# OpenVVC/OpenVVC

Hardware: AMD Instinct MI355X
Metric: decoded frames/sec, full rcn back-end decode step (H2D of the recorded picture + MC incl. BDOF/DMVR/affine-PROF/GPM/CIIP + LMCS + inverse transform + ordered intra pass + deblocking + SAO + ALF/CC-ALF + D2H of refined MVs + wait + per-picture digest + publication to the device DPB), 4K 10-bit RA rec (higher is better)
Workload: dtype u16 samples / int16 coefficients / int32 accumulate

## Files before the change

include/ovvc_hip.h:

```cpp
#ifndef OVVC_HIP_H
#define OVVC_HIP_H

#include <stddef.h>
#include <stdint.h>

#ifdef __cplusplus
extern "C" {
#endif

#define OVHIP_ABI_VERSION 9

#define OVHIP_OK        0
#define OVHIP_ENODEV   (-1)
#define OVHIP_ENOMEM   (-2)
#define OVHIP_EINVAL   (-3)
#define OVHIP_ELAUNCH  (-4)
#define OVHIP_EUNSUP   (-5)
#define OVHIP_EREF     (-6)

enum { OVHIP_DST_VII = 0, OVHIP_DCT_VIII = 1, OVHIP_DCT_II = 2 };

typedef struct ovhip_pic {
    uint16_t *y, *cb, *cr;
    int32_t   w, h;
// ... 557 lines not shown
                       const ovhip_aff_unit *d_aunits, uint32_t n_aunits, const int32_t *d_side,
                       const uint16_t *d_lmcs_fwd_lut);
#define OVHIP_INTRA_GEOM_ANY 0x12u
#define OVHIP_INTRA_GEOM_IBC 0x20u
uint32_t ovhip_intra_level_geom(const ovhip_itask *tasks, size_t n);
int  ovhip_intra_level_launch(ovhip_ctx *ctx, const ovhip_pic *pic, const ovhip_pic *res, const ovhip_itask *d_tasks, uint32_t n,
                              const ovhip_lmcs_region *d_regions, const ovhip_lmcs_luts *luts, int16_t *d_scales, int32_t log2_ctu_s,
                              uint32_t geom);
size_t ovhip_intra_sync_words(int32_t width, int32_t height, int32_t log2_ctu_s);
int  ovhip_intra_ctu_launch(ovhip_ctx *ctx, const ovhip_pic *pic, const ovhip_pic *res, const ovhip_itask *d_tasks, const ovhip_ictu *d_ctus,
                            uint32_t n_ctus, const ovhip_lmcs_region *d_regions, const ovhip_lmcs_luts *luts, int16_t *d_scales,
                            int32_t log2_ctu_s, uint32_t *d_sync, uint32_t epoch, uint32_t *abort_mirror);
#define OVHIP_FLOW_IBC 2
size_t ovhip_intra_flow_words(int32_t width, int32_t height);
size_t ovhip_intra_flow_items(const ovhip_itask *sorted, size_t n, uint32_t *items, size_t cap);
int  ovhip_intra_flow_launch(ovhip_ctx *ctx, const ovhip_pic *pic, const ovhip_pic *res, const ovhip_itask *d_tasks, uint32_t n_tasks,
                             const uint32_t *d_items, uint32_t n_items, const ovhip_lmcs_region *d_regions, const ovhip_lmcs_luts *luts,
                             int16_t *d_scales, int32_t log2_ctu_s, uint32_t *d_state, uint32_t epoch, uint32_t *abort_mirror, int32_t prepare,
                             int32_t n_workers);
int  ovhip_intra_flow_untag_launch(ovhip_ctx *ctx, const ovhip_pic *pic, const ovhip_itask *d_tasks, uint32_t n_tasks, int32_t with_luma);
int  ovhip_lmcs_scale_prepare_launch(ovhip_ctx *ctx, const ovhip_pic *pic, const ovhip_lmcs_region *d_regions, uint32_t n_regions,
                                     const ovhip_lmcs_luts *luts, int16_t *d_scales, const ovhip_itask *d_tasks, uint32_t n_tasks,
                                     uint32_t *d_state, uint32_t epoch);
int  ovhip_lmcs_inverse_untag_launch(ovhip_ctx *ctx, const ovhip_pic *pic, const uint16_t *d_bwd_lut, const ovhip_itask *d_tasks, uint32_t n_tasks);
int  ovhip_dbf_launch(ovhip_ctx *ctx, const ovhip_pic *pic, const ovhip_dbf_planes *planes);
int  ovhip_dbf_launch_edges(ovhip_ctx *ctx, const ovhip_pic *pic, const ovhip_dbf_edge *d_edges_v, uint32_t n_v,
                            const ovhip_dbf_edge *d_edges_h, uint32_t n_h, int32_t beta_offset, int32_t tc_offset);
int  ovhip_dbf_launch_edges_ex(ovhip_ctx *ctx, const ovhip_pic *pic, const ovhip_dbf_edge *d_edges_v, uint32_t n_v,
                               const ovhip_dbf_edge *d_edges_h, uint32_t n_h, const ovhip_dbf_offsets *offsets);
int  ovhip_sao_launch(ovhip_ctx *ctx, const ovhip_pic *dst, const ovhip_pic *src,
// ... 452 lines not shown
```

openvvc_amd/capi.py:

```python
from __future__ import annotations

import ctypes as C
import os
from pathlib import Path

import numpy as np

_PKG = Path(__file__).resolve().parent
LIB_PATH = _PKG / os.environ.get("OVVC_HIP_LIB_NAME", "libovvc_hip.so")

OVHIP_ABI_VERSION = 9
OVHIP_OK, OVHIP_ENODEV, OVHIP_ENOMEM, OVHIP_EINVAL, OVHIP_ELAUNCH, OVHIP_EUNSUP, OVHIP_EREF = 0, -1, -2, -3, -4, -5, -6
DST_VII, DCT_VIII, DCT_II = 0, 1, 2
TB_TR, TB_DC, TB_TS, TB_TS_RAW = 0, 1, 2, 3
TB_FLAG_RASTER = 0x80
RES_ADD, RES_SUB, RES_ADD_HALF, RES_SUB_HALF, RES_SCALE = 0, 1, 2, 3, 4
MC_HPEL_FILT, MC_FILT_4x4, MC_NO_LUMA, MC_NO_CHROMA, MC_LMCS, MC_BDOF, MC_DMVR = 1, 2, 4, 8, 16, 32, 64
PU_BDOF, PU_DMVR, PU_GPM = 1, 2, 4
MC_GPM = 128


class Pic(C.Structure):
    _fields_ = [("y", C.c_void_p), ("cb", C.c_void_p), ("cr", C.c_void_p),
                ("w", C.c_int32), ("h", C.c_int32), ("stride_y", C.c_int32), ("stride_c", C.c_int32)]
# ... 580 lines not shown
        "ovhip_mcx_launch": (C.c_int, [vp, P(Pic), P(Pic), u32, vp, u32, vp, vp]),
        "ovhip_mca_launch": (C.c_int, [vp, P(Pic), P(Pic), u32, vp, u32, vp, vp]),
        "ovhip_mcxa_launch": (C.c_int, [vp, P(Pic), P(Pic), u32, vp, u32, vp, vp, u32, vp, vp]),
        "ovhip_rec_create_ex": (vp, [i32, i32, vp]),
        "ovhip_rec_set_dense_dbf_planes": (None, [vp, C.c_int]),
        "ovhip_rec_dbf_edges": (vp, [vp, C.c_int, P(C.c_size_t), P(DbfOffsets)]),
        "ovhip_dbf_launch_edges_ex": (C.c_int, [vp, P(Pic), vp, u32, vp, u32, P(DbfOffsets)]),
        "ovhip_dmvr_search_launch": (C.c_int, [vp, P(Pic), P(Pic), u32, vp, u32, vp]),
        "ovhip_rec_append_raw": (C.c_int, [vp, C.c_int, vp, C.c_size_t]),
        "ovhip_itx_launch_classes_res": (C.c_int, [vp, P(Pic), P(Pic), vp, u32, u32, vp, vp]),
        "ovhip_intra_level_launch": (C.c_int, [vp, P(Pic), P(Pic), vp, u32, vp, vp, vp, i32, u32]),
        "ovhip_intra_level_geom": (u32, [vp, C.c_size_t]),
        "ovhip_intra_sync_words": (C.c_size_t, [i32, i32, i32]),
        "ovhip_intra_flow_words": (C.c_size_t, [i32, i32]),
        "ovhip_intra_flow_items": (C.c_size_t, [vp, C.c_size_t, vp, C.c_size_t]),
        "ovhip_intra_flow_launch": (C.c_int, [vp, P(Pic), P(Pic), vp, u32, vp, u32, vp, vp, vp, i32, vp, u32, vp, i32, i32]),
        "ovhip_intra_ctu_launch": (C.c_int, [vp, P(Pic), P(Pic), vp, vp, u32, vp, vp, vp, i32, vp, u32, vp]),
        "ovhip_rec_itask_levels": (u32, [vp]),
        "ovhip_rec_isp_cu": (C.c_int, [vp, vp, vp]),
        "ovhip_isp_geometry": (None, [i32, i32, i32, P(i32), P(i32), P(i32), P(i32)]),
        "ovhip_job_bind": (C.c_int, [vp, vp]),
        "ovhip_rec_set_ctu_size": (C.c_int, [vp, i32]),
        "ovhip_rec_itasks_by_ctu": (vp, [vp, i32, P(C.c_size_t), P(vp), P(C.c_size_t)]),
        "ovhip_rec_tu_intra": (C.c_int, [vp, P(TuState), P(TuDesc), P(ITask), P(ITask)]),
        "ovhip_rec_itasks": (vp, [vp, P(C.c_size_t)]),
        "ovhip_rec_ibc_check": (C.c_int, [vp, P(IbcDesc)]),
        "ovhip_rec_tu_ibc": (C.c_int, [vp, P(TuState), P(TuDesc), P(IbcDesc)]),
        "ovhip_rec_ibc_tasks": (C.c_size_t, [vp]),
        "ovhip_rec_itasks_sorted": (vp, [vp, P(C.c_size_t), P(P(C.c_uint32)), P(C.c_uint32)]),
        "ovhip_rec_set_dbf_offsets": (C.c_int, [vp, P(DbfOffsets), C.c_int]),
# ... 193 lines not shown
        raise RuntimeError("libovvc_hip.so ABI version mismatch")
    if path is None:
        _lib = lib
    return lib


EXPORTED_SYMBOLS = [
    "ovhip_abi_version", "ovhip_rec_create", "ovhip_rec_destroy", "ovhip_rec_reset", "ovhip_rec_tu",
    "ovhip_rec_pu", "ovhip_rec_cu_inter", "ovhip_rec_dbf_row", "ovhip_rec_dbf_mv_prepass_view", "ovhip_rec_dbf_ctu", "ovhip_rec_dbf_planes", "ovhip_dbf_launch", "ovhip_sao_launch", "ovhip_alf_launch", "ovhip_rec_tb_cmds", "ovhip_rec_coefs", "ovhip_rec_mc_units", "ovhip_rec_mcx_units", "ovhip_mcx_launch", "ovhip_rec_affine_cu", "ovhip_rec_transform_tree", "ovhip_rec_lmcs_region", "ovhip_dbf_compact", "ovhip_rec_dbf_mv_prepass", "ovhip_dbf_launch_edges", "ovhip_rec_ciip", "ovhip_ciip_weight", "ovhip_rec_ciip_units", "ovhip_ciip_launch", "ovhip_rec_lmcs_regions", "ovhip_rec_tb_cmds_split", "ovhip_itx_launch_classes", "ovhip_itx_launch_chroma_lmcs", "ovhip_lmcs_build", "ovhip_lmcs_scale_launch", "ovhip_lmcs_inverse_launch", "ovhip_rec_aff_units", "ovhip_rec_aff_side", "ovhip_mca_launch", "ovhip_mcxa_launch", "ovhip_ctx_create",
    "ovhip_ctx_destroy", "ovhip_ctx_sync", "ovhip_ctx_shares_queue", "ovhip_ctx_new_stream", "ovhip_ctx_fork", "ovhip_ctx_join", "ovhip_last_error", "ovhip_ctx_stream", "ovhip_malloc",
    "ovhip_free", "ovhip_h2d", "ovhip_d2h", "ovhip_pic_alloc", "ovhip_pic_free", "ovhip_pic_upload",
    "ovhip_pic_download", "ovhip_itx_launch", "ovhip_mc_launch",
    "ovhip_rec_set_ref_scale", "ovhip_rec_refusal", "ovhip_rec_rpr_units", "ovhip_mc_rpr_launch",
    "ovhip_rec_set_rpr_tools", "ovhip_rec_aff_rpr_units", "ovhip_mca_rpr_launch",
    "ovhip_rec_create_ex", "ovhip_rec_set_dense_dbf_planes", "ovhip_rec_dbf_edges", "ovhip_dbf_launch_edges_ex",
    "ovhip_dmvr_search_launch", "ovhip_rec_append_raw", "ovhip_rec_set_dbf_offsets", "ovhip_rec_tu_intra", "ovhip_rec_itasks", "ovhip_rec_itasks_sorted", "ovhip_itx_launch_classes_res", "ovhip_intra_level_launch", "ovhip_intra_level_geom", "ovhip_intra_sync_words", "ovhip_intra_ctu_launch", "ovhip_intra_flow_words", "ovhip_intra_flow_items", "ovhip_intra_flow_launch",
    "ovhip_rec_itask_levels", "ovhip_rec_isp_cu", "ovhip_isp_geometry", "ovhip_rec_itasks_by_ctu", "ovhip_rec_set_ctu_size", "ovhip_job_bind", "ovhip_job_create", "ovhip_job_destroy", "ovhip_job_recorder", "ovhip_job_begin",
    "ovhip_frame_band", "ovhip_frame_band_upto", "ovhip_frame_dmvr_rows_begin_upto", "ovhip_job_dmvr_rows_begin_upto", "ovhip_frame_set_band_mode", "ovhip_frame_band_stats", "ovhip_dpb_post_rows", "ovhip_dpb_rows_tag",
    "ovhip_job_band", "ovhip_job_band_active", "ovhip_job_band_busy", "ovhip_job_band_reserve", "ovhip_job_reserve_for_picture", "ovhip_rec_reserve_for_picture", "ovhip_job_band_progress", "ovhip_rec_counts", "ovhip_sao_launch_rows", "ovhip_alf_launch_rows",
    "ovhip_job_flush", "ovhip_job_wait", "ovhip_job_refined_mvs", "ovhip_job_dmvr_rows", "ovhip_job_dmvr_rows_begin", "ovhip_job_dmvr_rows_collect", "ovhip_job_last_stats", "ovhip_job_time_stage", "ovhip_job_stage_time",
    "ovhip_output_bytes", "ovhip_output_rows", "ovhip_output_pack_launch", "ovhip_output_row_md5_launch", "ovhip_output_bands", "ovhip_output_tree_md5_launch", "ovhip_pic_output", "ovhip_pic_digest",
    "ovhip_md5_init", "ovhip_md5_update", "ovhip_md5_final", "ovhip_tmvp_cells_launch", "ovhip_job_tmvp_cells", "ovhip_intra_flow_untag_launch", "ovhip_lmcs_inverse_untag_launch", "ovhip_lmcs_scale_prepare_launch",
    "ovhip_host_alloc", "ovhip_host_free", "ovhip_d2d", "ovhip_job_test_abort_next_flow",
    "ovhip_dpb_create", "ovhip_dpb_create_ex", "ovhip_dpb_destroy", "ovhip_dpb_n_devices", "ovhip_dpb_device", "ovhip_dpb_begin", "ovhip_dpb_want",
    "ovhip_dpb_publish", "ovhip_dpb_acquire", "ovhip_dpb_wait_copy", "ovhip_dpb_poll_tag", "ovhip_frame_refs_ready", "ovhip_dpb_set_unknown_key_timeout", "ovhip_dpb_unpin", "ovhip_dpb_release", "ovhip_dpb_lookup", "ovhip_dpb_shutdown",
    "ovhip_dpb_get_stats", "ovhip_dpb_begin_tag", "ovhip_dpb_want_tag", "ovhip_dpb_acquire_tag", "ovhip_frame_begin_tag", "ovhip_frame_ref_tag", "ovhip_frame_set_trace",
    "ovhip_rccl_unique_id", "ovhip_rccl_create", "ovhip_rccl_destroy", "ovhip_rccl_xfer", "ovhip_rccl_last_error", "ovhip_rccl_stats", "ovhip_rccl_self_exchange",
    "ovhip_frame_create", "ovhip_frame_destroy", "ovhip_frame_ctx", "ovhip_frame_job", "ovhip_frame_recorder", "ovhip_frame_begin", "ovhip_frame_ref",
    "ovhip_frame_ref_at", "ovhip_frame_dmvr_rows", "ovhip_frame_dmvr_rows_begin", "ovhip_frame_dmvr_rows_collect", "ovhip_frame_submit", "ovhip_frame_fail", "ovhip_frame_last_error",
    "ovhip_calllog_create", "ovhip_calllog_destroy", "ovhip_calllog_reset", "ovhip_calllog_data", "ovhip_rec_set_calllog", "ovhip_calllog_replay",
    "ovhip_stream_create", "ovhip_stream_destroy", "ovhip_stream_run", "ovhip_stream_frame", "ovhip_stream_key", "ovhip_stream_queue_info",
# ... 280 lines not shown
```

openvvc_amd/csrc/flow_state.hip.h:

```cpp
#pragma once
#include <hip/hip_runtime.h>
#include <stdint.h>
#include "ovvc_hip.h"

#define OVHIP_FLOW_SYNC_WORDS 16
struct FlowState { unsigned *y, *c[2], *reg; int w4; };

static inline FlowState flow_state_of(uint32_t *d_state, int w, int h)
{
    FlowState fs;
    const size_t nu = (size_t)((w + 3) / 4) * ((h + 3) / 4);
    fs.w4 = (w + 3) / 4;
    fs.y = d_state + OVHIP_FLOW_SYNC_WORDS; fs.c[0] = fs.y + nu; fs.c[1] = fs.c[0] + nu; fs.reg = fs.c[1] + nu;
    return fs;
}

#define FLOW_ITEM_TASK_BITS  24
#define FLOW_ITEM_STRIP_BITS 5
#define FLOW_ITEM_MAX_TASKS  ((size_t)1 << FLOW_ITEM_TASK_BITS)
#define FLOW_ITEM_MAX_STRIPS (1 << FLOW_ITEM_STRIP_BITS)
struct FlowItem { uint32_t task; int strip, plane; };

__host__ __device__ static inline uint32_t flow_item_pack(uint32_t task, int strip, int plane)
{
    return task | ((uint32_t)strip << FLOW_ITEM_TASK_BITS) | ((uint32_t)plane << (FLOW_ITEM_TASK_BITS + FLOW_ITEM_STRIP_BITS));
}
__host__ __device__ static inline FlowItem flow_item_unpack(uint32_t word)
{
    FlowItem it;
    it.task = word & ((1u << FLOW_ITEM_TASK_BITS) - 1);
    it.strip = (int)((word >> FLOW_ITEM_TASK_BITS) & (FLOW_ITEM_MAX_STRIPS - 1));
    it.plane = (int)((word >> (FLOW_ITEM_TASK_BITS + FLOW_ITEM_STRIP_BITS)) & 1);
    return it;
}

extern "C" size_t ovhip_intra_flow_items_(const ovhip_itask *sorted, size_t n, uint32_t *items, size_t cap);

__device__ __forceinline__ void flow_prepare_task(const ovhip_itask &t, const FlowState &fs, unsigned epoch, int lane16)
{
    const unsigned mark = 2 * epoch;
    if (t.kind == OVHIP_IT_REGION) { if (lane16 == 0) fs.reg[t.c_scale] = mark; return; }
    const bool luma = t.kind == OVHIP_IT_LUMA || t.kind == OVHIP_IT_IBC_L;
    const bool both = t.kind == OVHIP_IT_CHROMA || t.kind == OVHIP_IT_IBC_C;
    const int sh = luma ? 2 : 1, w = 1 << t.log2_w, h = 1 << t.log2_h;
    const int ux0 = t.x >> sh, uy0 = t.y >> sh, nx = max(1, w >> sh), ny = max(1, h >> sh);
    const int l2nx = 31 - __clz(nx);
    for (int i = lane16; i < nx * ny; i += 16) {
        const int u = (uy0 + (i >> l2nx)) * fs.w4 + ux0 + (i & (nx - 1));
        if (luma) fs.y[u] = mark;
        else {
// ... 6 lines not shown
```

openvvc_amd/csrc/kernels_intra.hip:

```cpp
#include <stdlib.h>
#include "ovvc_common.hip.h"
#include "flow_state.hip.h"
#include "lmcs_wnd.hip.h"
#define OVT_ATTR __device__
#include "vvc_mip_tables.h"

namespace {

__device__ const short g_ang[32] = { 0, 1, 2, 3, 4, 6, 8, 10, 12, 14, 16, 18, 20, 23, 26, 29, 32, 35, 39, 45, 51, 57, 64, 73, 86, 102, 128, 171, 256, 341, 512, 1024 };
__device__ const short g_inv_ang[32] = { 0, 16384, 8192, 5461, 4096, 2731, 2048, 1638, 1365, 1170, 1024, 910, 819, 712, 630, 565, 512, 468, 420, 364,
                                         321, 287, 256, 224, 191, 161, 128, 96, 64, 48, 32, 16 };
__device__ __attribute__((aligned(4))) const signed char g_fc[32][4] = {
    { 0, 64, 0, 0 }, { -1, 63, 2, 0 }, { -2, 62, 4, 0 }, { -2, 60, 7, -1 }, { -2, 58, 10, -2 }, { -3, 57, 12, -2 }, { -4, 56, 14, -2 },
    { -4, 55, 15, -2 }, { -4, 54, 16, -2 }, { -5, 53, 18, -2 }, { -6, 52, 20, -2 }, { -6, 49, 24, -3 }, { -6, 46, 28, -4 }, { -5, 44, 29, -4 },
    { -4, 42, 30, -4 }, { -4, 39, 33, -4 }, { -4, 36, 36, -4 }, { -4, 33, 39, -4 }, { -4, 30, 42, -4 }, { -4, 29, 44, -5 }, { -4, 28, 46, -6 },
    { -3, 24, 49, -6 }, { -2, 20, 52, -6 }, { -2, 18, 53, -5 }, { -2, 16, 54, -4 }, { -2, 15, 55, -4 }, { -2, 14, 56, -4 }, { -2, 12, 57, -3 },
    { -2, 10, 58, -2 }, { -1, 7, 60, -2 }, { 0, 4, 62, -2 }, { 0, 2, 63, -1 } };

#define IR_NEG  64
#define IR_TAIL 48
#define IR_LEN  (IR_NEG + 2 * 64 + 4 + IR_TAIL)
struct IntraLds {
    uint16_t abv[IR_LEN], lft[IR_LEN];
    uint16_t fabv[IR_LEN], flft[IR_LEN];
// ... 951 lines not shown
                if (it.scaled) for (int e = 0; e < G; ++e) v[e] = ov_clip_bd(v[e] + res_scale(rv[e], scale));
                else           for (int e = 0; e < G; ++e) v[e] = ov_clip_bd(v[e] + rv[e]);
            }
#pragma unroll
            for (int e = 0; e < R::DW; ++e) out[e] = ((uint32_t)v[2 * e] | (G > 1 ? (uint32_t)v[G > 1 ? 2 * e + 1 : 0] << 16 : 0u)) | tag2;
        }
        uint16_t *o = dst + y * dstride + x;
        if constexpr (G == 8) asm volatile("global_store_dwordx4 %0, %1, off sc1" :: "v"(o), "v"(out) : "memory");
        else if constexpr (G == 4) asm volatile("global_store_dwordx2 %0, %1, off sc1" :: "v"(o), "v"(out) : "memory");
        else __hip_atomic_store(o, (uint16_t)out[0], RLX_AGENT);
    }
}

struct FlowLds { IntraLds s; uint32_t fp[FLOW_MAX_FP]; int abort; };

template <bool IBC>
__global__ __launch_bounds__(64) void k_intra_flow(ovhip_pic pic, ovhip_pic res, const ovhip_itask *__restrict__ tasks, const uint32_t *__restrict__ items,
                                                   uint32_t n_items, const ovhip_lmcs_region *__restrict__ regs, LmcsWnd wnd, int16_t *scales,
                                                   int log2_ctu, FlowState fs, unsigned epoch, unsigned *sync, unsigned *abort_mirror)
{
    __shared__ FlowLds L;
    IntraLds &s = L.s;
    if (blockIdx.x >= n_items) return;
    __builtin_amdgcn_s_setprio(OVHIP_FLOW_PRIO);
    const int lane = threadIdx.x;
    load_tables(s, lane);
    int prev_level = 0;
    for (uint32_t bid = blockIdx.x; bid < n_items; bid += gridDim.x) {
    if (bid != blockIdx.x) wave_sync();
    FPROBE_DECL;
    const FlowItem fi = flow_item_unpack(items[bid]);
    const ovhip_itask t = tasks[fi.task];
    const int comp = fi.plane;
    const Item it = item_of<FSTRIP, IBC>(t, fi.strip, comp);
    const int l2w = t.log2_w, w = 1 << l2w, h = 1 << t.log2_h;
    const bool luma = it.luma;
    const bool ibc = IBC && t.kind >= OVHIP_IT_IBC_L;
    const unsigned pending = 2 * epoch;
    const int w4 = fs.w4;
    if (it.skip()) continue;

    uint16_t *pl = luma ? pic.y : (comp ? pic.cr : pic.cb);
    const int dstride = luma ? pic.stride_y : pic.stride_c, rstride = luma ? res.stride_y : res.stride_c;
    uint16_t *dst = pl + t.y * dstride + t.x;
    const int16_t *rp = reinterpret_cast<const int16_t *>(luma ? res.y : (comp ? res.cr : res.cb)) + t.y * rstride + t.x;
    const int run = w >= 8 ? 8 : (w == 4 ? 4 : 1);
    FlowRaw raw = { };
// ... 188 lines not shown
    if (!ctx || !pic || !res) return OVHIP_EINVAL;
    OV_DEVICE(ctx);
    if (!n_ctus) return OVHIP_OK;
    if (!d_tasks || !d_ctus || !d_sync || !epoch || log2_ctu_s < 5 || log2_ctu_s > 7)
        return ov_fail(ctx, OVHIP_EINVAL, "ovhip_intra_ctu_launch: bad arguments", hipSuccess);
    if ((pic->w & 7) || (pic->h & 1) || (pic->stride_y & 3) || (pic->stride_c & 3) || ((uintptr_t)pic->y & 7) || ((uintptr_t)pic->cb & 7) || ((uintptr_t)pic->cr & 7))
        return ov_fail(ctx, OVHIP_EUNSUP, "ovhip_intra_ctu_launch: picture width must be a multiple of 8 and the planes 8-byte aligned", hipSuccess);
    const LmcsWnd wnd = lmcs_wnd_of(luts);
    const int ncx = (pic->w + (1 << log2_ctu_s) - 1) >> log2_ctu_s;
    hipLaunchKernelGGL(k_intra_ctu, dim3(n_ctus), dim3(256), 0, ctx->stream, *pic, *res, d_tasks, d_ctus, d_regions, wnd, d_scales, log2_ctu_s, d_sync, epoch, ncx,
                       abort_mirror);
    OV_LAUNCH_CHECK(ctx, "k_intra_ctu");
    return OVHIP_OK;
}

extern "C" size_t ovhip_intra_flow_items_(const ovhip_itask *sorted, size_t n, uint32_t *items, size_t cap)
{
    size_t k = 0;
    for (size_t i = 0; sorted && i < n; ++i) {
        const ovhip_itask &t = sorted[i];
        if (i >= FLOW_ITEM_MAX_TASKS) return 0;
        if (t.kind == OVHIP_IT_REGION) { if (k < cap) items[k] = flow_item_pack((uint32_t)i, 0, 0); ++k; continue; }
        const int npx = 1 << (t.log2_w + t.log2_h), strips = (npx + FSTRIP - 1) / FSTRIP, comps = (t.kind == OVHIP_IT_LUMA || t.kind == OVHIP_IT_IBC_L) ? 1 : 2;
        if (strips > FLOW_ITEM_MAX_STRIPS) return 0;
        for (int st = 0; st < strips; ++st)
            for (int c = 0; c < comps; ++c) { if (k < cap) items[k] = flow_item_pack((uint32_t)i, st, c); ++k; }
    }
    return k;
}

extern "C" size_t ovhip_intra_flow_items(const ovhip_itask *sorted, size_t n, uint32_t *items, size_t cap)
{
    const size_t k = ovhip_intra_flow_items_(sorted, n, items, cap);
    return k <= cap ? k : 0;
}

extern "C" size_t ovhip_intra_flow_words(int32_t width, int32_t height)
{
    if (width <= 0 || height <= 0) return 0;
    return SYNC_FLAGS + 4 * (size_t)((width + 3) / 4) * ((height + 3) / 4);
}

extern "C" int ovhip_intra_flow_launch(ovhip_ctx *ctx, const ovhip_pic *pic, const ovhip_pic *res, const ovhip_itask *d_tasks, uint32_t n_tasks,
                                       const uint32_t *d_items, uint32_t n_items, const ovhip_lmcs_region *d_regions, const ovhip_lmcs_luts *luts,
                                       int16_t *d_scales, int32_t log2_ctu_s, uint32_t *d_state, uint32_t epoch, uint32_t *abort_mirror, int32_t prepare,
                                       int32_t n_workers)
{
    if (!ctx || !pic || !res) return OVHIP_EINVAL;
// ... 35 lines not shown
```

openvvc_amd/csrc/ovvc_band.hip:

```cpp
#include "ovvc_job.hip.h"

extern "C" void ovhip_rec_tb_split_range_(const ovhip_recorder *r, size_t first, size_t n, ovhip_tb_cmd *out, size_t counts[4], size_t tiny[4][4]);
extern "C" int  ovhip_rec_itasks_sorted_range_(const ovhip_recorder *r, size_t first, size_t n, ovhip_itask *out, uint32_t *level_start, size_t cap, uint32_t *n_levels);

enum { MAX_BANDS = 96, ARENA_CHUNKS = 16, BAND_LEVELS = 4096 };
struct ArenaChunk { char *host, *dev; size_t cap, used; };
struct BandRec {
    int32_t row0, row1;
    ovhip_band_counts c0, c1;
    const ovhip_itask *d_it; uint32_t n_it; int tagged;
    const ovhip_dbf_edge *d_ev, *d_eh; uint32_t n_ev, n_eh;
    int flow_charge;
    int32_t rows_final;
};
struct BandState {
    int active, n, tails, closed, failed;
    ovhip_pic dst;
    ovhip_band_counts cur;
    int32_t row_prev, dbf_rows, sao_rows, alf_rows, rows_final;
    int log2_ctu, sao_on, alf_on, filters_latched;
    uint32_t stages;
    const uint16_t *d_fwd, *d_bwd; int lmcs_up;
    ovhip_alf_pic d_alf; int alf_up;
    ovhip_lmcs_luts luts; int have_luts;
// ... 256 lines not shown
    const size_t o_tb = L.put(n.n_tb * sizeof(ovhip_tb_cmd)), o_coef = L.put((size_t)n.n_coef * 2), o_mc = L.put(n.n_mc * sizeof(ovhip_mc_unit)),
                 o_mcx = L.put(n.n_mcx * sizeof(ovhip_mc_unit)), o_aff = L.put(n.n_aff * sizeof(ovhip_aff_unit)), o_side = L.put((size_t)n.n_side * 4),
                 o_reg = L.put(n.n_reg * sizeof(ovhip_lmcs_region)), o_it = L.put(n.n_itask * sizeof(ovhip_itask)), o_items = L.put(k.n_items * 4),
                 o_ev = L.put(n.n_edge_v * sizeof(ovhip_dbf_edge)), o_eh = L.put(n.n_edge_h * sizeof(ovhip_dbf_edge));
    p.o_sao = L.put(k.n_sao * sizeof(ovhip_sao_ctu)); p.o_alf = L.put(k.n_alf * sizeof(ovhip_alf_ctu));
    const size_t upload_bytes = L.o;
    const size_t o_mv = L.put((size_t)n.n_mcx * 16);
    char *hb = nullptr, *db = nullptr;
    if (L.o) CHK(arena_take(j, L.o, &hb, &db));

    uint32_t n_lv = 0;
    if (n.n_tb) ovhip_rec_tb_split_range_(rec, c0.n_tb, n.n_tb, (ovhip_tb_cmd *)(hb + o_tb), c.cls, c.tiny);
    k.have_levels = n.n_itask && ovhip_rec_itasks_sorted_range_(rec, c0.n_itask, n.n_itask, (ovhip_itask *)(hb + o_it), bs->level_start, BAND_LEVELS + 2, &n_lv) == 0;
    if (n.n_itask && !k.have_levels && !k.n_items) return ov_fail(ctx, OVHIP_EUNSUP, "ovhip_job_band: a band with more levels than the table holds and blocks the flow launch cannot take", hipSuccess);
    k.h_items = (const uint32_t *)(hb + o_items);
    if (k.n_items) (void)ovhip_intra_flow_items_((const ovhip_itask *)(hb + o_it), n.n_itask, (uint32_t *)(hb + o_items), k.n_items);
    size_t all;
    if (n.n_coef) memcpy(hb + o_coef, ovhip_rec_coefs(rec, &all) + c0.n_coef, (size_t)n.n_coef * 2);
    if (n.n_mc) memcpy(hb + o_mc, ovhip_rec_mc_units(rec, &all) + c0.n_mc, n.n_mc * sizeof(ovhip_mc_unit));
    if (n.n_mcx) memcpy(hb + o_mcx, ovhip_rec_mcx_units(rec, &all) + c0.n_mcx, n.n_mcx * sizeof(ovhip_mc_unit));
    if (n.n_aff) memcpy(hb + o_aff, ovhip_rec_aff_units(rec, &all) + c0.n_aff, n.n_aff * sizeof(ovhip_aff_unit));
    if (n.n_side) memcpy(hb + o_side, ovhip_rec_aff_side(rec, &all) + c0.n_side, (size_t)n.n_side * 4);
    if (n.n_reg) memcpy(hb + o_reg, ovhip_rec_lmcs_regions(rec, &all) + c0.n_reg, n.n_reg * sizeof(ovhip_lmcs_region));
    const ovhip_dbf_edge *ev = ovhip_rec_dbf_edges(rec, 0, &all, &bs->offs), *eh = ovhip_rec_dbf_edges(rec, 1, &all, nullptr);
    if (n.n_edge_v) memcpy(hb + o_ev, ev + c0.n_edge_v, n.n_edge_v * sizeof(ovhip_dbf_edge));
    if (n.n_edge_h) memcpy(hb + o_eh, eh + c0.n_edge_h, n.n_edge_h * sizeof(ovhip_dbf_edge));
    if (k.n_sao) memcpy(hb + p.o_sao, pr->sao + (size_t)k.sao_r0 * k.nb_ctu_w, k.n_sao * sizeof(ovhip_sao_ctu));
    if (k.n_alf) memcpy(hb + p.o_alf, pr->alf_ctus + (size_t)k.alf_r0 * k.nb_ctu_w, k.n_alf * sizeof(ovhip_alf_ctu));
    tables_fill(hb, p.tabs, pr, alf_now, lmcs_now);
    if (upload_bytes) {
        OV_HIP(ctx, hipMemcpyAsync(db, hb, upload_bytes, hipMemcpyHostToDevice, ctx->stream));
// ... 124 lines not shown
```

openvvc_amd/csrc/ovvc_record_intra.c:

```c
#include <stdlib.h>
#include <string.h>
#include "ovvc_hip.h"
#include "ovvc_record_priv.h"

static int
maps_ready(ovhip_recorder *r)
{
    const int w4 = (r->pic_w + 3) >> 2, h4 = (r->pic_h + 3) >> 2;
    if (!r->lvl_y) {
        r->lvl_y = (uint16_t *)calloc((size_t)w4 * h4, 2);
        r->lvl_c = (uint16_t *)calloc((size_t)w4 * h4, 2);
        if (!r->lvl_y || !r->lvl_c) return -1;
        r->lvl_w4 = w4; r->lvl_h4 = h4; r->lvl_dirty = 0;
    }
    if (r->lvl_dirty) {
        memset(r->lvl_y, 0, (size_t)w4 * h4 * 2); memset(r->lvl_c, 0, (size_t)w4 * h4 * 2);
        r->lvl_dirty = 0;
    }
    return 0;
}

int
ovhip_rec_intra_reset_(ovhip_recorder *r)
{
// ... 148 lines not shown
{
    if (!r) return 0;
    uint32_t m = r->max_ilevel;
    if (!m) for (size_t i = 0; i < r->n_itask; ++i) if (r->itask[i].level > m) m = r->itask[i].level;
    return m;
}

const ovhip_itask *
ovhip_rec_itasks(const ovhip_recorder *r, size_t *n)
{
    if (!r || !n) return NULL;
    *n = r->n_itask;
    return r->itask;
}

const ovhip_itask *
ovhip_rec_itasks_sorted(ovhip_recorder *r, size_t *n, const uint32_t **level_start, uint32_t *n_levels)
{
    if (!r || !n || !level_start || !n_levels) return NULL;
    *n = r->n_itask; *n_levels = 0; *level_start = NULL;
    if (!r->n_itask) return r->itask;
    uint32_t maxl = 0;
    for (size_t i = 0; i < r->n_itask; ++i) if (r->itask[i].level > maxl) maxl = r->itask[i].level;
    if (ovhip_rec_grow_(r, (void **)&r->itask_sorted, &r->cap_isorted, r->n_itask, sizeof(ovhip_itask))) { *n = 0; return NULL; }
    {
        if (r->cap_ilevel < (size_t)(maxl + 2) * 2) {
            uint32_t *q = (uint32_t *)realloc(r->ilevel_start, (size_t)(maxl + 2) * 2 * sizeof(uint32_t));
            if (!q) { *n = 0; return NULL; }
            r->ilevel_start = q; r->cap_ilevel = (size_t)(maxl + 2) * 2;
        }
    }
    uint32_t *start = r->ilevel_start;
    memset(start, 0, (maxl + 2) * sizeof(uint32_t));
    for (size_t i = 0; i < r->n_itask; ++i) start[r->itask[i].level]++;
    uint32_t acc = 0;
    for (uint32_t l = 1; l <= maxl; ++l) { const uint32_t c = start[l]; start[l] = acc; acc += c; }
    start[maxl + 1] = acc;
    uint32_t *fill = start + maxl + 2;
    memcpy(fill, start, (maxl + 2) * sizeof(uint32_t));
    for (size_t i = 0; i < r->n_itask; ++i) r->itask_sorted[fill[r->itask[i].level]++] = r->itask[i];
    r->n_ilevels = maxl;
    *n_levels = maxl;
    *level_start = start + 1;
    return r->itask_sorted;
}

int
ovhip_rec_itasks_sorted_range_(const ovhip_recorder *r, size_t first, size_t n, ovhip_itask *out, uint32_t *level_start, size_t cap, uint32_t *n_levels)
{
    *n_levels = 0;
    if (!n) return 0;
    const ovhip_itask *t = r->itask + first;
    uint32_t minl = 0xffffffffu, maxl = 0;
    for (size_t i = 0; i < n; ++i) { if (t[i].level < minl) minl = t[i].level; if (t[i].level > maxl) maxl = t[i].level; }
    const size_t span = (size_t)(maxl - minl) + 1;
    uint32_t *cnt = (uint32_t *)calloc(span + 1, sizeof(uint32_t));
    if (!cnt) return -1;
    for (size_t i = 0; i < n; ++i) cnt[t[i].level - minl]++;
    uint32_t acc = 0, nl = 0;
    int fits = 1;
    for (size_t l = 0; l < span; ++l) {
        const uint32_t c = cnt[l];
        cnt[l] = acc;
        if (c) { if (nl < cap) level_start[nl] = acc; else fits = 0; ++nl; }
        acc += c;
    }
    if (nl < cap) level_start[nl] = acc; else fits = 0;
    for (size_t i = 0; i < n; ++i) out[cnt[t[i].level - minl]++] = t[i];
    free(cnt);
    *n_levels = nl;
    return fits ? 0 : -1;
}

const ovhip_itask *
ovhip_rec_itasks_by_ctu(ovhip_recorder *r, int32_t log2_ctu_s, size_t *n, const ovhip_ictu **ctus, size_t *n_ctus)
{
    if (!r || !n || !ctus || !n_ctus || log2_ctu_s < 5 || log2_ctu_s > 7) return NULL;
    *n = 0; *ctus = NULL; *n_ctus = 0;
    if (!r->n_itask) return r->itask;
    const uint32_t *lv; uint32_t nlv; size_t nt;
    const ovhip_itask *sorted = ovhip_rec_itasks_sorted(r, &nt, &lv, &nlv);
    if (!sorted) return NULL;
    const int ncx = (r->pic_w + (1 << log2_ctu_s) - 1) >> log2_ctu_s, ncy = (r->pic_h + (1 << log2_ctu_s) - 1) >> log2_ctu_s;
// ... 54 lines not shown
```

openvvc_amd/engine.py:

```python
from __future__ import annotations

import ctypes as C

import numpy as np

from . import capi


class EngineError(RuntimeError):
    pass


def rgb_format(matrix: int = 1, full_range: int = 0, chroma_loc: int = 0, dtype: int = capi.RGB_U8, layout: int = capi.RGB_PLANAR) -> capi.RgbFormat:
    return capi.RgbFormat(matrix, full_range, chroma_loc, dtype, layout)


def rgb_shape(fmt: capi.RgbFormat, w: int, h: int, window=(0, 0, 0, 0)) -> tuple:
    W, H = w - 2 * (window[0] + window[1]), h - 2 * (window[2] + window[3])
    return (3, H, W) if fmt.layout == capi.RGB_PLANAR else (H, W, 3)


def _device_tensor(tensor, what: str, dtypes: tuple, shape: "tuple | None" = None, need: "int | None" = None, slots: bool = False) -> "tuple[int, int, int]":
    import torch
    if not isinstance(tensor, torch.Tensor) or not tensor.is_cuda:
# ... 242 lines not shown
                    luts=None, scales: "DevBuf | None" = None, log2_ctu: int = 7, geom: int = 0x12):
        ptr = C.c_void_p(tasks.ptr.value + first * 32)
        self._chk(self.lib.ovhip_intra_level_launch(self.h, C.byref(pic.s), C.byref(res.s), ptr, n, regions.ptr if regions else None,
                                                    C.byref(luts) if luts is not None else None, scales.ptr if scales else None, log2_ctu, geom),
                  "intra_level_launch")

    def intra_ctu(self, pic: "DevPic", res: "DevPic", tasks: "DevBuf", ctus: "DevBuf", n_ctus: int, sync: "DevBuf", epoch: int,
                  regions: "DevBuf | None" = None, luts=None, scales: "DevBuf | None" = None, log2_ctu: int = 7):
        self._chk(self.lib.ovhip_intra_ctu_launch(self.h, C.byref(pic.s), C.byref(res.s), tasks.ptr, ctus.ptr, n_ctus,
                                                  regions.ptr if regions else None, C.byref(luts) if luts is not None else None,
                                                  scales.ptr if scales else None, log2_ctu, sync.ptr, epoch, None), "intra_ctu_launch")

    def intra_flow_words(self, w: int, h: int) -> int:
        return int(self.lib.ovhip_intra_flow_words(w, h))

    def intra_flow_items(self, tasks: np.ndarray) -> np.ndarray:
        tasks = np.ascontiguousarray(tasks)
        items = np.zeros(32 * len(tasks), np.uint32)
        n = int(self.lib.ovhip_intra_flow_items(tasks.ctypes.data, len(tasks), items.ctypes.data, len(items)))
        if len(tasks) and not n:
            raise EngineError("intra_flow_items: the flow launch cannot take this task list")
        return items[:n]

    def intra_flow(self, pic: "DevPic", res: "DevPic", tasks: "DevBuf", n_tasks: int, items: "DevBuf", n_items: int, state: "DevBuf",
                   epoch: int, regions: "DevBuf | None" = None, luts=None, scales: "DevBuf | None" = None, log2_ctu: int = 7,
                   prepare: int = 1, n_workers: int = 0):
        self._chk(self.lib.ovhip_intra_flow_launch(self.h, C.byref(pic.s), C.byref(res.s), tasks.ptr, n_tasks, items.ptr, n_items,
                                                   regions.ptr if regions else None, C.byref(luts) if luts is not None else None,
                                                   scales.ptr if scales else None, log2_ctu, state.ptr, epoch, None, prepare, n_workers),
                  "intra_flow_launch")

    def intra_flow_abort(self, state: "DevBuf") -> int:
        self.sync()
        word = np.zeros(1, np.uint32)
# ... 1054 lines not shown
```

Before: 3635.

## Batch same-level chroma residual tasks into run items in intra flow kernel

```diff
diff --git a/include/ovvc_hip.h b/include/ovvc_hip.h
--- a/include/ovvc_hip.h
+++ b/include/ovvc_hip.h
@@ -595,6 +595,7 @@
 #define OVHIP_FLOW_IBC 2
 size_t ovhip_intra_flow_words(int32_t width, int32_t height);
 size_t ovhip_intra_flow_items(const ovhip_itask *sorted, size_t n, uint32_t *items, size_t cap);
+size_t ovhip_intra_flow_items_runs(const ovhip_itask *sorted, size_t n, uint32_t *items, size_t cap);
 int  ovhip_intra_flow_launch(ovhip_ctx *ctx, const ovhip_pic *pic, const ovhip_pic *res, const ovhip_itask *d_tasks, uint32_t n_tasks,
                              const uint32_t *d_items, uint32_t n_items, const ovhip_lmcs_region *d_regions, const ovhip_lmcs_luts *luts,
                              int16_t *d_scales, int32_t log2_ctu_s, uint32_t *d_state, uint32_t epoch, uint32_t *abort_mirror, int32_t prepare,
diff --git a/openvvc_amd/capi.py b/openvvc_amd/capi.py
--- a/openvvc_amd/capi.py
+++ b/openvvc_amd/capi.py
@@ -618,6 +618,7 @@
         "ovhip_intra_sync_words": (C.c_size_t, [i32, i32, i32]),
         "ovhip_intra_flow_words": (C.c_size_t, [i32, i32]),
         "ovhip_intra_flow_items": (C.c_size_t, [vp, C.c_size_t, vp, C.c_size_t]),
+        "ovhip_intra_flow_items_runs": (C.c_size_t, [vp, C.c_size_t, vp, C.c_size_t]),
         "ovhip_intra_flow_launch": (C.c_int, [vp, P(Pic), P(Pic), vp, u32, vp, u32, vp, vp, vp, i32, vp, u32, vp, i32, i32]),
         "ovhip_intra_ctu_launch": (C.c_int, [vp, P(Pic), P(Pic), vp, vp, u32, vp, vp, vp, i32, vp, u32, vp]),
         "ovhip_rec_itask_levels": (u32, [vp]),
@@ -841,7 +842,7 @@
     "ovhip_rec_set_ref_scale", "ovhip_rec_refusal", "ovhip_rec_rpr_units", "ovhip_mc_rpr_launch",
     "ovhip_rec_set_rpr_tools", "ovhip_rec_aff_rpr_units", "ovhip_mca_rpr_launch",
     "ovhip_rec_create_ex", "ovhip_rec_set_dense_dbf_planes", "ovhip_rec_dbf_edges", "ovhip_dbf_launch_edges_ex",
-    "ovhip_dmvr_search_launch", "ovhip_rec_append_raw", "ovhip_rec_set_dbf_offsets", "ovhip_rec_tu_intra", "ovhip_rec_itasks", "ovhip_rec_itasks_sorted", "ovhip_itx_launch_classes_res", "ovhip_intra_level_launch", "ovhip_intra_level_geom", "ovhip_intra_sync_words", "ovhip_intra_ctu_launch", "ovhip_intra_flow_words", "ovhip_intra_flow_items", "ovhip_intra_flow_launch",
+    "ovhip_dmvr_search_launch", "ovhip_rec_append_raw", "ovhip_rec_set_dbf_offsets", "ovhip_rec_tu_intra", "ovhip_rec_itasks", "ovhip_rec_itasks_sorted", "ovhip_itx_launch_classes_res", "ovhip_intra_level_launch", "ovhip_intra_level_geom", "ovhip_intra_sync_words", "ovhip_intra_ctu_launch", "ovhip_intra_flow_words", "ovhip_intra_flow_items", "ovhip_intra_flow_items_runs", "ovhip_intra_flow_launch",
     "ovhip_rec_itask_levels", "ovhip_rec_isp_cu", "ovhip_isp_geometry", "ovhip_rec_itasks_by_ctu", "ovhip_rec_set_ctu_size", "ovhip_job_bind", "ovhip_job_create", "ovhip_job_destroy", "ovhip_job_recorder", "ovhip_job_begin",
     "ovhip_frame_band", "ovhip_frame_band_upto", "ovhip_frame_dmvr_rows_begin_upto", "ovhip_job_dmvr_rows_begin_upto", "ovhip_frame_set_band_mode", "ovhip_frame_band_stats", "ovhip_dpb_post_rows", "ovhip_dpb_rows_tag",
     "ovhip_job_band", "ovhip_job_band_active", "ovhip_job_band_busy", "ovhip_job_band_reserve", "ovhip_job_reserve_for_picture", "ovhip_rec_reserve_for_picture", "ovhip_job_band_progress", "ovhip_rec_counts", "ovhip_sao_launch_rows", "ovhip_alf_launch_rows",
diff --git a/openvvc_amd/csrc/flow_state.hip.h b/openvvc_amd/csrc/flow_state.hip.h
--- a/openvvc_amd/csrc/flow_state.hip.h
+++ b/openvvc_amd/csrc/flow_state.hip.h
@@ -34,6 +34,20 @@
     return it;
 }
 
+#define FLOW_ITEM_RUN        0x80000000u
+#define FLOW_ITEM_RUN_MAX    (1 << (FLOW_ITEM_STRIP_BITS + 1))
+#define FLOW_ITEM_RUN_LEN(word) ((int)(((word) >> FLOW_ITEM_TASK_BITS) & (FLOW_ITEM_RUN_MAX - 1)) + 1)
+
+__host__ __device__ static inline uint32_t flow_item_pack_run(uint32_t first, int len)
+{
+    return FLOW_ITEM_RUN | first | ((uint32_t)(len - 1) << FLOW_ITEM_TASK_BITS);
+}
+__host__ __device__ static inline bool flow_run_mates(const ovhip_itask &a, const ovhip_itask &b)
+{
+    const int sf = OVHIP_IF_RES_SCALE | OVHIP_IF_SCALE_IDX;
+    return a.kind == OVHIP_IT_RES_C && b.kind == OVHIP_IT_RES_C && !((a.flags | b.flags) & OVHIP_IF_ISP) && a.level == b.level && a.c_scale == b.c_scale && !((a.flags ^ b.flags) & sf);
+}
+
 extern "C" size_t ovhip_intra_flow_items_(const ovhip_itask *sorted, size_t n, uint32_t *items, size_t cap);
 
 __device__ __forceinline__ void flow_prepare_task(const ovhip_itask &t, const FlowState &fs, unsigned epoch, int lane16)
diff --git a/openvvc_amd/csrc/kernels_intra.hip b/openvvc_amd/csrc/kernels_intra.hip
--- a/openvvc_amd/csrc/kernels_intra.hip
+++ b/openvvc_amd/csrc/kernels_intra.hip
@@ -989,6 +989,105 @@
 
 struct FlowLds { IntraLds s; uint32_t fp[FLOW_MAX_FP]; int abort; };
 
+struct FlowResPlanes { uint16_t *cb, *cr; const int16_t *rcb, *rcr; int stride, rstride; unsigned *state_cb, *state_cr, *state_reg; int w4; };
+
+__device__ __forceinline__ void flow_res_narrow(const IntraLds &s, const ovhip_itask &t, int scale, const FlowResPlanes pl, int lane)
+{
+    const int l2w = t.log2_w, strips = ((1 << (t.log2_w + t.log2_h)) + FSTRIP - 1) / FSTRIP;
+    const int off = t.y * pl.stride + t.x, roff = t.y * pl.rstride + t.x;
+    for (int st = 0; st < strips; ++st) {
+        const Item a = item_of<FSTRIP>(t, st, 0), b = item_of<FSTRIP>(t, st, 1);
+        FlowRaw qa = { }, qb = { };
+        if (!a.skip()) flow_load<1>(qa, a, pl.cb + off, pl.stride, pl.rcb + roff, pl.rstride, l2w, lane);
+        if (!b.skip()) flow_load<1>(qb, b, pl.cr + off, pl.stride, pl.rcr + roff, pl.rstride, l2w, lane);
+        if (!a.skip()) flow_store<1>(s, qa, a, scale, pl.cb + off, pl.stride, l2w, lane);
+        if (!b.skip()) flow_store<1>(s, qb, b, scale, pl.cr + off, pl.stride, l2w, lane);
+    }
+}
+
+#define FLOW_RUN_BATCH 4
+__device__ __forceinline__ bool flow_res_run(FlowLds &L, const ovhip_itask *__restrict__ tasks, uint32_t first, int n, const ovhip_itask &t0,
+                                             const FlowResPlanes pl, const int16_t *scales, unsigned pending, unsigned *sync, int lane)
+{
+    const bool scaled = t0.flags & OVHIP_IF_RES_SCALE, by_idx = scaled && (t0.flags & OVHIP_IF_SCALE_IDX);
+    uint32_t xy = 0, geo = 0, nq = 0;
+    if (lane < n) {
+        const ovhip_itask *t = tasks + first + lane;
+        const uint32_t l2w = t->log2_w, l2h = t->log2_h, flags = t->flags;
+        xy = (uint32_t)t->x | (uint32_t)t->y << 16;
+        geo = l2w | l2h << 8 | flags << 16;
+        const uint32_t planes = ((flags & OVHIP_IF_RES_CB) ? 1u : 0u) + ((flags & OVHIP_IF_RES_CR) ? 1u : 0u);
+        nq = l2w >= 2 ? planes << (l2w + l2h - 2) : 0;
+    }
+    int scale = scaled ? (int)t0.c_scale : 0;
+    if (by_idx) {
+        unsigned *f = pl.state_reg + t0.c_scale;
+        unsigned spins = 0;
+        unsigned cur = __builtin_amdgcn_readfirstlane(__hip_atomic_load(f, RLX_AGENT));
+        while (cur == pending) {
+            if (++spins > SPIN_LIMIT) return false;
+            __builtin_amdgcn_s_sleep(4);
+            const unsigned stop = __builtin_amdgcn_readfirstlane(__hip_atomic_load(sync, RLX_AGENT));
+            cur = __builtin_amdgcn_readfirstlane(__hip_atomic_load(f, RLX_AGENT));
+            if (stop != 0) return false;
+        }
+        scale = (int)__hip_atomic_load(scales + t0.c_scale, RLX_AGENT);
+    }
+    uint32_t incl = nq;
+#pragma unroll
+    for (int d = 1; d < 64; d <<= 1) { const uint32_t v = __shfl_up(incl, d); if (lane >= d) incl += v; }
+    const uint32_t total = __shfl(incl, 63);
+    L.fp[lane] = incl - nq; L.fp[64 + lane] = xy; L.fp[128 + lane] = geo;
+    wave_sync();
+    for (unsigned long long narrow = __ballot(lane < n && (geo & 0xff) < 2); narrow; narrow &= narrow - 1)
+        flow_res_narrow(L.s, tasks[first + (uint32_t)__builtin_ctzll(narrow)], scale, pl, lane);
+    for (uint32_t base = 0; base < total; base += 64 * FLOW_RUN_BATCH) {
+        FlowRaw raw[FLOW_RUN_BATCH];
+        uint16_t *dst[FLOW_RUN_BATCH];
+        int p0[FLOW_RUN_BATCH], l2w[FLOW_RUN_BATCH];
+        auto item = [&](int p, bool valid) {
+            Item it;
+            it.luma = false; it.region = false; it.res_only = true; it.lm = false; it.has_res = valid; it.scaled = scaled; it.scale_idx = by_idx;
+            it.ciip_wt = 0; it.res_mask = 0xff; it.res_l2pb = 6; it.p0 = p; it.p1 = p + 4;
+            return it;
+        };
+#pragma unroll
+        for (int b = 0; b < FLOW_RUN_BATCH; ++b) {
+            const uint32_t q = base + 64 * b + lane;
+            int k = 0;
+#pragma unroll
+            for (int st = 32; st; st >>= 1) { const int c = k + st; if (c < n && L.fp[c] <= q) k = c; }
+            const uint32_t txy = L.fp[64 + k], g = L.fp[128 + k], flags = g >> 16;
+            uint32_t lq = q - L.fp[k];
+            l2w[b] = (int)(g & 0xff);
+            const uint32_t per_plane = 1u << (l2w[b] + ((g >> 8) & 0xff) - 2);
+            const bool both = (flags & OVHIP_IF_RES_CB) && (flags & OVHIP_IF_RES_CR);
+            const bool cr = both ? lq >= per_plane : !(flags & OVHIP_IF_RES_CB);
+            if (both && cr) lq -= per_plane;
+            p0[b] = q < total ? (int)(lq << 2) : -1;
+            const int off = (int)(txy >> 16) * pl.stride + (int)(txy & 0xffff), roff = (int)(txy >> 16) * pl.rstride + (int)(txy & 0xffff);
+            dst[b] = (cr ? pl.cr : pl.cb) + off;
+            raw[b] = FlowRaw{ };
+            if (p0[b] >= 0) flow_load<4>(raw[b], item(p0[b], true), dst[b], pl.stride, (cr ? pl.rcr : pl.rcb) + roff, pl.rstride, l2w[b], 0);
+        }
+#pragma unroll
+        for (int b = 0; b < FLOW_RUN_BATCH; ++b)
+            if (p0[b] >= 0) flow_store<4>(L.s, raw[b], item(p0[b], true), scale, dst[b], pl.stride, l2w[b], 0);
+    }
+    asm volatile("s_waitcnt vmcnt(0)" ::: "memory");
+    for (int k = 0; k < n; ++k) {
+        const uint32_t txy = L.fp[64 + k], g = L.fp[128 + k], flags = g >> 16;
+        const int ux0 = (int)(txy & 0xffff) >> 1, uy0 = (int)(txy >> 16) >> 1, nx = max(1, (1 << (g & 0xff)) >> 1), ny = max(1, (1 << ((g >> 8) & 0xff)) >> 1);
+        const int l2nx = ilog2(nx);
+        for (int i = lane; i < nx * ny; i += 64) {
+            const int u = (uy0 + (i >> l2nx)) * pl.w4 + ux0 + (i & (nx - 1));
+            if (flags & OVHIP_IF_RES_CB) __hip_atomic_store(pl.state_cb + u, pending + 1, RLX_AGENT);
+            if (flags & OVHIP_IF_RES_CR) __hip_atomic_store(pl.state_cr + u, pending + 1, RLX_AGENT);
+        }
+    }
+    return true;
+}
+
 template <bool IBC>
 __global__ __launch_bounds__(64) void k_intra_flow(ovhip_pic pic, ovhip_pic res, const ovhip_itask *__restrict__ tasks, const uint32_t *__restrict__ items,
                                                    uint32_t n_items, const ovhip_lmcs_region *__restrict__ regs, LmcsWnd wnd, int16_t *scales,
@@ -1004,8 +1103,22 @@
     for (uint32_t bid = blockIdx.x; bid < n_items; bid += gridDim.x) {
     if (bid != blockIdx.x) wave_sync();
     FPROBE_DECL;
-    const FlowItem fi = flow_item_unpack(items[bid]);
+    const uint32_t word = items[bid];
+    const FlowItem fi = flow_item_unpack(word);
     const ovhip_itask t = tasks[fi.task];
+    if (word & FLOW_ITEM_RUN) {
+        const int gap = min((int)t.level - prev_level - 1, FLOW_NAP_MAX_LEVELS);
+        prev_level = (int)t.level;
+        if (gap > 0) {
+            __builtin_amdgcn_s_setprio(0);
+            for (int k = 0; k < 2 * gap; ++k) __builtin_amdgcn_s_sleep(FLOW_NAP_HALF_LEVEL);
+            __builtin_amdgcn_s_setprio(OVHIP_FLOW_PRIO);
+        }
+        const FlowResPlanes rp = { pic.cb, pic.cr, reinterpret_cast<const int16_t *>(res.cb), reinterpret_cast<const int16_t *>(res.cr), pic.stride_c, res.stride_c,
+                                   fs.c[0], fs.c[1], fs.reg, fs.w4 };
+        if (!flow_res_run(L, tasks, fi.task, FLOW_ITEM_RUN_LEN(word), t, rp, scales, 2 * epoch, sync, lane)) { flow_give_up(sync, abort_mirror, lane); return; }
+        continue;
+    }
     const int comp = fi.plane;
     const Item it = item_of<FSTRIP, IBC>(t, fi.strip, comp);
     const int l2w = t.log2_w, w = 1 << l2w, h = 1 << t.log2_h;
@@ -1224,7 +1337,7 @@
     return OVHIP_OK;
 }
 
-extern "C" size_t ovhip_intra_flow_items_(const ovhip_itask *sorted, size_t n, uint32_t *items, size_t cap)
+static size_t flow_items(const ovhip_itask *sorted, size_t n, uint32_t *items, size_t cap, bool runs)
 {
     size_t k = 0;
     for (size_t i = 0; sorted && i < n; ++i) {
@@ -1233,15 +1346,35 @@
         if (t.kind == OVHIP_IT_REGION) { if (k < cap) items[k] = flow_item_pack((uint32_t)i, 0, 0); ++k; continue; }
         const int npx = 1 << (t.log2_w + t.log2_h), strips = (npx + FSTRIP - 1) / FSTRIP, comps = (t.kind == OVHIP_IT_LUMA || t.kind == OVHIP_IT_IBC_L) ? 1 : 2;
         if (strips > FLOW_ITEM_MAX_STRIPS) return 0;
+        if (runs && t.kind == OVHIP_IT_RES_C && !(t.flags & OVHIP_IF_ISP)) {
+            size_t e = i + 1;
+            for (; e < n && e < FLOW_ITEM_MAX_TASKS && e - i < FLOW_ITEM_RUN_MAX && flow_run_mates(t, sorted[e]); ++e)
+                if (((1 << (sorted[e].log2_w + sorted[e].log2_h)) + FSTRIP - 1) / FSTRIP > FLOW_ITEM_MAX_STRIPS) return 0;
+            if (k < cap) items[k] = flow_item_pack_run((uint32_t)i, (int)(e - i));
+            ++k;
+            i = e - 1;
+            continue;
+        }
         for (int st = 0; st < strips; ++st)
             for (int c = 0; c < comps; ++c) { if (k < cap) items[k] = flow_item_pack((uint32_t)i, st, c); ++k; }
     }
     return k;
 }
 
+extern "C" size_t ovhip_intra_flow_items_(const ovhip_itask *sorted, size_t n, uint32_t *items, size_t cap)
+{
+    return flow_items(sorted, n, items, cap, true);
+}
+
 extern "C" size_t ovhip_intra_flow_items(const ovhip_itask *sorted, size_t n, uint32_t *items, size_t cap)
 {
-    const size_t k = ovhip_intra_flow_items_(sorted, n, items, cap);
+    const size_t k = flow_items(sorted, n, items, cap, false);
+    return k <= cap ? k : 0;
+}
+
+extern "C" size_t ovhip_intra_flow_items_runs(const ovhip_itask *sorted, size_t n, uint32_t *items, size_t cap)
+{
+    const size_t k = flow_items(sorted, n, items, cap, true);
     return k <= cap ? k : 0;
 }
 
diff --git a/openvvc_amd/csrc/ovvc_band.hip b/openvvc_amd/csrc/ovvc_band.hip
--- a/openvvc_amd/csrc/ovvc_band.hip
+++ b/openvvc_amd/csrc/ovvc_band.hip
@@ -294,7 +294,11 @@
     k.have_levels = n.n_itask && ovhip_rec_itasks_sorted_range_(rec, c0.n_itask, n.n_itask, (ovhip_itask *)(hb + o_it), bs->level_start, BAND_LEVELS + 2, &n_lv) == 0;
     if (n.n_itask && !k.have_levels && !k.n_items) return ov_fail(ctx, OVHIP_EUNSUP, "ovhip_job_band: a band with more levels than the table holds and blocks the flow launch cannot take", hipSuccess);
     k.h_items = (const uint32_t *)(hb + o_items);
-    if (k.n_items) (void)ovhip_intra_flow_items_((const ovhip_itask *)(hb + o_it), n.n_itask, (uint32_t *)(hb + o_items), k.n_items);
+    if (k.n_items) {
+        const size_t cap = k.n_items;
+        k.n_items = ovhip_intra_flow_items_((const ovhip_itask *)(hb + o_it), n.n_itask, (uint32_t *)(hb + o_items), cap);
+        if (k.n_items > cap) return ov_fail(ctx, OVHIP_EINVAL, "ovhip_job_band: more flow items after the sort than before it", hipSuccess);
+    }
     size_t all;
     if (n.n_coef) memcpy(hb + o_coef, ovhip_rec_coefs(rec, &all) + c0.n_coef, (size_t)n.n_coef * 2);
     if (n.n_mc) memcpy(hb + o_mc, ovhip_rec_mc_units(rec, &all) + c0.n_mc, n.n_mc * sizeof(ovhip_mc_unit));
diff --git a/openvvc_amd/csrc/ovvc_record_intra.c b/openvvc_amd/csrc/ovvc_record_intra.c
--- a/openvvc_amd/csrc/ovvc_record_intra.c
+++ b/openvvc_amd/csrc/ovvc_record_intra.c
@@ -186,6 +186,36 @@
     return r->itask;
 }
 
+#define RES_C_KEY(t) ((uint32_t)(uint16_t)(t).c_scale * 4u + (((uint32_t)(t).flags / OVHIP_IF_RES_SCALE) & 3u))
+static uint32_t *
+res_c_order(const ovhip_itask *t, size_t n)
+{
+    size_t nres = 0;
+    uint32_t kmin = 0xffffffffu, kmax = 0;
+    for (size_t i = 0; i < n; ++i) {
+        if (t[i].kind != OVHIP_IT_RES_C) continue;
+        const uint32_t k = RES_C_KEY(t[i]);
+        if (k < kmin) kmin = k;
+        if (k > kmax) kmax = k;
+        ++nres;
+    }
+    if (nres < 2) return NULL;
+    const size_t span = (size_t)(kmax - kmin) + 1;
+    uint32_t *ord = (uint32_t *)malloc((n + span) * sizeof(uint32_t));
+    if (!ord) return NULL;
+    uint32_t *cnt = ord + n;
+    memset(cnt, 0, span * sizeof(uint32_t));
+    for (size_t i = 0; i < n; ++i) if (t[i].kind == OVHIP_IT_RES_C) cnt[RES_C_KEY(t[i]) - kmin]++;
+    uint32_t acc = (uint32_t)(n - nres);
+    for (size_t k = 0; k < span; ++k) { const uint32_t c = cnt[k]; cnt[k] = acc; acc += c; }
+    uint32_t pos = 0;
+    for (size_t i = 0; i < n; ++i) {
+        if (t[i].kind == OVHIP_IT_RES_C) ord[cnt[RES_C_KEY(t[i]) - kmin]++] = (uint32_t)i;
+        else ord[pos++] = (uint32_t)i;
+    }
+    return ord;
+}
+
 const ovhip_itask *
 ovhip_rec_itasks_sorted(ovhip_recorder *r, size_t *n, const uint32_t **level_start, uint32_t *n_levels)
 {
@@ -210,7 +240,9 @@
     start[maxl + 1] = acc;
     uint32_t *fill = start + maxl + 2;
     memcpy(fill, start, (maxl + 2) * sizeof(uint32_t));
-    for (size_t i = 0; i < r->n_itask; ++i) r->itask_sorted[fill[r->itask[i].level]++] = r->itask[i];
+    uint32_t *ord = res_c_order(r->itask, r->n_itask);
+    for (size_t i = 0; i < r->n_itask; ++i) { const ovhip_itask *q = &r->itask[ord ? ord[i] : i]; r->itask_sorted[fill[q->level]++] = *q; }
+    free(ord);
     r->n_ilevels = maxl;
     *n_levels = maxl;
     *level_start = start + 1;
@@ -238,7 +270,9 @@
         acc += c;
     }
     if (nl < cap) level_start[nl] = acc; else fits = 0;
-    for (size_t i = 0; i < n; ++i) out[cnt[t[i].level - minl]++] = t[i];
+    uint32_t *ord = res_c_order(t, n);
+    for (size_t i = 0; i < n; ++i) { const ovhip_itask *q = &t[ord ? ord[i] : i]; out[cnt[q->level - minl]++] = *q; }
+    free(ord);
     free(cnt);
     *n_levels = nl;
     return fits ? 0 : -1;
diff --git a/openvvc_amd/engine.py b/openvvc_amd/engine.py
--- a/openvvc_amd/engine.py
+++ b/openvvc_amd/engine.py
@@ -280,10 +280,11 @@
     def intra_flow_words(self, w: int, h: int) -> int:
         return int(self.lib.ovhip_intra_flow_words(w, h))
 
-    def intra_flow_items(self, tasks: np.ndarray) -> np.ndarray:
+    def intra_flow_items(self, tasks: np.ndarray, runs: bool = False) -> np.ndarray:
         tasks = np.ascontiguousarray(tasks)
         items = np.zeros(32 * len(tasks), np.uint32)
-        n = int(self.lib.ovhip_intra_flow_items(tasks.ctypes.data, len(tasks), items.ctypes.data, len(items)))
+        fn = self.lib.ovhip_intra_flow_items_runs if runs else self.lib.ovhip_intra_flow_items
+        n = int(fn(tasks.ctypes.data, len(tasks), items.ctypes.data, len(items)))
         if len(tasks) and not n:
             raise EngineError("intra_flow_items: the flow launch cannot take this task list")
         return items[:n]
```

After: 3614. No clear change (-0.6%).
